# ipc-sim/IPC

Measured on NVIDIA H100. Metric: newton_iteration_ms_assembly_ccd, lower is better.
Workload: dtype f64

## Files before the change

### ipc_b200/csrc/api_mesh.cu

```cuda
#include "abi.h"
#include <algorithm>
#include <cmath>
#include <numeric>
#include <vector>

using namespace ipcgpu;

int build_maps(ipcgpu_ctx* ctx)
{
    const int nT = ctx->nT, nV = ctx->nV;
    const std::vector<int>& T = ctx->h_T;
    ctx->t_begin = (int)((int64_t)nT * ctx->rank / ctx->nranks);
    ctx->t_end = (int)((int64_t)nT * (ctx->rank + 1) / ctx->nranks);
    std::vector<int64_t> cum(nV + 1, 0);
    for (size_t i = 0; i < (size_t)4 * nT; ++i) ++cum[T[i] + 1];
    for (int v = 0; v < nV; ++v) cum[v + 1] += cum[v];
    auto boundary = [&](int r) -> int {
        if (r <= 0) return 0;
        if (r >= ctx->nranks) return nV;
        const int64_t target = cum[nV] * r / ctx->nranks;
        return (int)(std::lower_bound(cum.begin(), cum.end(), target) - cum.begin());
    };
    const int vb = std::min(boundary(ctx->rank), nV), ve = std::max(vb, std::min(boundary(ctx->rank + 1), nV));
    ctx->v_begin = vb;
    ctx->v_end = ve;
    std::vector<int> list;
    if (ctx->nranks == 1) {
        list.resize(nT);
        std::iota(list.begin(), list.end(), 0);
    }
    else {
        list.reserve((size_t)(nT / ctx->nranks) + 1024);
        for (int t = 0; t < nT; ++t) {
            bool touch = false;
            for (int k = 0; k < 4; ++k) {
                const int v = T[(size_t)k * nT + t];
                touch = touch || (v >= vb && v < ve);
            }
            if (touch) list.push_back(t);
        }
    }
    const int nL = (int)list.size();
    ctx->n_list = nL;
    if (list.empty()) list.push_back(0);
    REQUIRE(ctx->tet_list.upload(list.data(), list.size(), ctx->stream), IPCGPU_ERR_CUDA, "upload of the tet list failed");
    std::vector<int> ptr(nV + 1, 0);
    for (int l = 0; l < nL; ++l)
        for (int k = 0; k < 4; ++k) {
            const int v = T[(size_t)k * nT + list[l]];
            if (v >= vb && v < ve) ++ptr[v + 1];
        }
    for (int v = 0; v < nV; ++v) ptr[v + 1] += ptr[v];
    std::vector<int> inc((size_t)std::max(ptr[nV], 1)), cur(ptr.begin(), ptr.end() - 1);
    for (int l = 0; l < nL; ++l)
        for (int k = 0; k < 4; ++k) {
            const int v = T[(size_t)k * nT + list[l]];
            if (v >= vb && v < ve) inc[cur[v]++] = 4 * l + k;
        }
    if (!ctx->inc_ptr.upload(ptr.data(), ptr.size(), ctx->stream) || !ctx->inc.upload(inc.data(), inc.size(), ctx->stream)) {
        ctx->err = "upload of incidence map failed";
        return IPCGPU_ERR_CUDA;
    }
    REQUIRE(((uint64_t)nL + 64ull) * 78ull < 0xffffffffull, IPCGPU_ERR_CAPACITY, "local tet count too large for 32-bit block offsets");
    struct KS {
        uint64_t key;
        unsigned src;
        unsigned tet;
    };
    std::vector<KS> ks;
    ks.reserve((size_t)10 * nL);
    static const int pa[6] = { 0, 0, 0, 1, 1, 2 }, pb[6] = { 1, 2, 3, 2, 3, 3 };
    for (int l = 0; l < nL; ++l) {
        const int t = list[l];
        int v[4];
        for (int k = 0; k < 4; ++k) v[k] = T[(size_t)k * nT + t];
        const unsigned tl = (unsigned)l, tile_base = (tl / 64u) * (64u * 78u), tin = tl % 64u;
        for (int a = 0; a < 4; ++a)
            if (v[a] >= vb && v[a] < ve) ks.push_back({ ((uint64_t)v[a] << 32) | (uint32_t)v[a], tile_base + 6u * a * 64u + tin * 6u, tl });
        for (int q = 0; q < 6; ++q) {
            const int lo = std::min(v[pa[q]], v[pb[q]]), hi = std::max(v[pa[q]], v[pb[q]]);
            if (lo >= vb && lo < ve) ks.push_back({ ((uint64_t)lo << 32) | (uint32_t)hi, tile_base + (24u + 9u * q) * 64u + tin * 9u, tl });
        }
    }
    std::sort(ks.begin(), ks.end(), [](const KS& a, const KS& b) { return a.key < b.key || (a.key == b.key && (a.tet < b.tet || (a.tet == b.tet && a.src < b.src))); });
    std::vector<int> sv, su, cptr;
    std::vector<unsigned> csrc(std::max<size_t>(ks.size(), 1));
    for (size_t i = 0; i < ks.size(); ++i) {
        if (i == 0 || ks[i].key != ks[i - 1].key) {
            sv.push_back((int)(ks[i].key >> 32));
            su.push_back((int)(ks[i].key & 0xffffffffu));
            cptr.push_back((int)i);
        }
        csrc[i] = ks[i].src;
    }
    cptr.push_back((int)ks.size());
    {
        const size_t nS = sv.size();
        std::vector<int> order;
        order.reserve(nS);
        for (size_t i = 0; i < nS; ++i)
            if (sv[i] != su[i]) order.push_back((int)i);
        ctx->nOffSlots = (int)order.size();
        for (size_t i = 0; i < nS; ++i)
            if (sv[i] == su[i]) order.push_back((int)i);
        std::vector<int> sv2(nS), su2(nS), cptr2;
        std::vector<unsigned> csrc2(csrc.size());
        cptr2.reserve(nS + 1);
        size_t pos = 0;
        for (size_t k = 0; k < nS; ++k) {
            const int i = order[k];
            sv2[k] = sv[i];
            su2[k] = su[i];
            cptr2.push_back((int)pos);
            for (int c = cptr[i]; c < cptr[i + 1]; ++c) csrc2[pos++] = csrc[c];
        }
        cptr2.push_back((int)pos);
        sv.swap(sv2); su.swap(su2); cptr.swap(cptr2); csrc.swap(csrc2);
    }
    ctx->nSlots = (int)sv.size();
    if (sv.empty()) { sv.push_back(0); su.push_back(0); }
    bool ok = ctx->slot_v.upload(sv.data(), sv.size(), ctx->stream) && ctx->slot_u.upload(su.data(), su.size(), ctx->stream)
        && ctx->con_ptr.upload(cptr.data(), cptr.size(), ctx->stream) && ctx->con_src.upload(csrc.data(), csrc.size(), ctx->stream)
        && ctx->slot_off.reserve((size_t)3 * std::max(1, ctx->nSlots));
    REQUIRE(ok, IPCGPU_ERR_CUDA, "upload of Hessian scatter map failed");
    ALLOC(ctx->gcont, (size_t)12 * std::max(1, nL));
    ALLOC(ctx->hblk, (size_t)78 * 64 * ((size_t)(std::max(1, nL) + 63) / 64));
    ALLOC(ctx->partials, (size_t)std::max(1, elastic_energy_blocks(ctx->t_end - ctx->t_begin)) + 8);
    CK(cudaStreamSynchronize(ctx->stream));
    ctx->maps_ready = true;
    ctx->offsets_ready = false;
    ctx->damp_on = ctx->damp_inc_ready = ctx->nbc_on = false;
    ctx->n_dbc = 0;
    for (int slot : { kEnergyDamping, kEnergyNeumann, kEnergyDirichlet })
        CK(cudaMemsetAsync(&ctx->iter.p->energy[slot], 0, sizeof(double), ctx->stream));
    CK(cudaStreamSynchronize(ctx->stream));
    return IPCGPU_OK;
}

void owned_value_range(ipcgpu_ctx* ctx)
{
    if (ctx->h_ia.empty()) return;
    ctx->a_begin = (long long)ctx->h_ia[(size_t)3 * ctx->v_begin] - ctx->index_base;
    ctx->a_end = (long long)ctx->h_ia[(size_t)3 * ctx->v_end] - ctx->index_base;
}

int ensure_offsets(ipcgpu_ctx* ctx)
{
    if (ctx->offsets_ready) return IPCGPU_OK;
    REQUIRE(ctx->maps_ready, IPCGPU_ERR_STATE, "ipcgpu_set_mesh must precede Hessian assembly");
    REQUIRE(ctx->n_rows == 3 * ctx->nV, IPCGPU_ERR_STATE, "ipcgpu_set_csr must be called with n_rows = 3*nV");
    CK(cudaMemsetAsync(ctx->flag.p, 0, sizeof(int), ctx->stream));
    slot_offsets(ctx->nSlots, ctx->slot_v.p, ctx->slot_u.p, ctx->ia.p, ctx->ja.p, ctx->index_base, ctx->slot_off.p, ctx->flag.p, ctx->stream);
    ++ctx->launches;
    int h = 0;
    CK(cudaMemcpyAsync(&h, ctx->flag.p, sizeof(int), cudaMemcpyDeviceToHost, ctx->stream));
    CK(cudaStreamSynchronize(ctx->stream));
    REQUIRE(h == 0, IPCGPU_ERR_PATTERN, "CSR pattern misses a block of the mesh topology (row<=col entries of every tet vertex pair are required)");
    ctx->offsets_ready = true;
    return IPCGPU_OK;
}

int upload_dir(ipcgpu_ctx* ctx, const double* p)
{
    if (p) {
        CK(cudaMemcpyAsync(ctx->dir.p, p, (size_t)3 * ctx->nV * sizeof(double), cudaMemcpyHostToDevice, ctx->stream));
        double pSize = 0;
        int nMeshSV = 0;
        for (int i = 0; i < ctx->nSV; ++i) {
            const int v = ctx->h_SVI[i];
            if (v >= ctx->nVdof) continue;
            ++nMeshSV;
            pSize += std::abs(p[3 * (size_t)v]);
            pSize += std::abs(p[3 * (size_t)v + 1]);
            pSize += std::abs(p[3 * (size_t)v + 2]);
        }
        ctx->pSize = nMeshSV > 0 ? pSize / (double)((long long)nMeshSV * 3) : 0.0;
        ALLOC(ctx->pSize_dev, 1);
        ctx->staging->pSize = ctx->pSize;
        CK(cudaMemcpyAsync(ctx->pSize_dev.p, &ctx->staging->pSize, sizeof(double), cudaMemcpyHostToDevice, ctx->stream));
        ctx->pSize_surface = ctx->surface_ready;
        ctx->dir_valid = true;
    }
    REQUIRE(ctx->dir_valid, IPCGPU_ERR_STATE, "no search direction uploaded yet");
    return IPCGPU_OK;
}
// ... 76 lines not shown
int ipcgpu_save_state(ipcgpu_ctx* ctx)
{
    REQUIRE(ctx->nV > 0, IPCGPU_ERR_STATE, "ipcgpu_set_mesh first");
    ENTER(kSerial);
    CK(cudaMemcpyAsync(ctx->Vsaved.p, ctx->V.p, (size_t)3 * ctx->nV * sizeof(double), cudaMemcpyDeviceToDevice, ctx->stream));
    ctx->state_saved = true;
    return IPCGPU_OK;
}

int ipcgpu_set_search_dir(ipcgpu_ctx* ctx, const double* p)
{
    REQUIRE(ctx->nV > 0 && p, IPCGPU_ERR_ARG, "ipcgpu_set_search_dir: mesh and p required");
    ENTER(kSerial);
    return upload_dir(ctx, p);
}

int ipcgpu_step_forward(ipcgpu_ctx* ctx, const double* p, double alpha)
{
    REQUIRE(ctx->nV > 0, IPCGPU_ERR_STATE, "ipcgpu_set_mesh first");
    REQUIRE(ctx->state_saved, IPCGPU_ERR_STATE, "ipcgpu_save_state must precede ipcgpu_step_forward");
    ENTER(kSerial);
    int rc = upload_dir(ctx, p);
    if (rc) return rc;
    step_forward(ctx->nV, ctx->Vsaved.p, ctx->dir.p, alpha, ctx->V.p, ctx->stream);
    ++ctx->launches;
    CK(cudaGetLastError());
    ctx->mark_inputs();
    return IPCGPU_OK;
}

int ipcgpu_elastic_energy(ipcgpu_ctx* ctx, double coef, int , double* E)
{
    REQUIRE(ctx->maps_ready, IPCGPU_ERR_STATE, "ipcgpu_set_mesh first");
    ENTER(kSerial);
    cudaEvent_t pe = ctx->prof_begin(IPCGPU_STAGE_ELASTIC_ENERGY);
    elastic_energy(ctx->eargs(), ctx->e_per_tet.p, ctx->partials.p, ctx->stream);
    return energy_tail(ctx, kEnergyElastic, ctx->partials.p, elastic_energy_blocks(ctx->t_end - ctx->t_begin), coef, pe, E);
}

static int zero_values(ipcgpu_ctx* ctx)
{
    cudaStream_t st = ctx->deriv_stream();
    if (ctx->device_pattern) {
        const bool owned = ctx->nranks > 1 && !ctx->a_all_dirty;
        zero_csr_rows(ctx->ia.p, ctx->index_base, owned ? 3 * ctx->v_begin : 0, owned ? 3 * ctx->v_end : 3 * ctx->nV, ctx->a.p, st);
    }
    else if (ctx->nranks > 1 && !ctx->a_all_dirty) {
        if (ctx->a_end > ctx->a_begin) zero_words(ctx->a.p + ctx->a_begin, (size_t)(ctx->a_end - ctx->a_begin) * 2, st);
    }
    else zero_words(ctx->a.p, (size_t)ctx->nnz * 2, st);
    ++ctx->launches;
    CK(cudaGetLastError());
    ctx->a_all_dirty = false;
    return IPCGPU_OK;
}

static int run_grad_hess(ipcgpu_ctx* ctx, double coef, int projectSPD, int projectDBC, bool need_g, bool need_h, int add_mass, bool with_energy = false,
    bool cleared = false)
{
    REQUIRE(ctx->maps_ready, IPCGPU_ERR_STATE, "ipcgpu_set_mesh first");
    if (need_h) {
        int rc = ensure_offsets(ctx);
        if (rc) return rc;
    }
    cudaStream_t st = ctx->deriv_stream();
    cudaEvent_t pe = ctx->prof_begin(IPCGPU_STAGE_ELASTIC_TET);
    double* e_part = nullptr;
    if (with_energy) {
        ALLOC(ctx->e_partials2, (size_t)elastic_grad_hess_blocks(ctx->n_list) + 8);
        e_part = ctx->e_partials2.p;
    }
    elastic_grad_hess(ctx->eargs(), coef, projectSPD, need_g, need_h, ctx->gcont.p, ctx->hblk.p, st, e_part);
    ctx->hblk_valid = need_h;
    ctx->prof_end(pe);
    ++ctx->launches;
    if (with_energy) {
        pe = ctx->prof_begin(IPCGPU_STAGE_ELASTIC_ENERGY);
        reduce_sum(e_part, elastic_grad_hess_blocks(ctx->n_list), coef, &ctx->iter.p->energy[kEnergyElastic], st);
        ctx->prof_end(pe);
        ++ctx->launches;
    }
    if (need_g) {
        pe = ctx->prof_begin(IPCGPU_STAGE_GATHER_GRADIENT);
        gather_gradient(ctx->nV, ctx->inc_ptr.p, ctx->inc.p, ctx->gcont.p, ctx->has_dbc ? ctx->dbc.p : nullptr, projectDBC, 0, ctx->g.p, st);
        ctx->prof_end(pe);
        ++ctx->launches;
    }
    if (need_h) {
        pe = ctx->prof_begin(IPCGPU_STAGE_ASSEMBLE_CSR);
        assemble_csr(ctx->nOffSlots, ctx->nSlots, ctx->slot_v.p, ctx->slot_u.p, ctx->slot_off.p, ctx->con_ptr.p, ctx->con_src.p, ctx->hblk.p,
            ctx->has_dbc ? ctx->dbc.p : nullptr, projectDBC, nullptr, cleared ? 0 : 1, ctx->a.p, st);
        const double* m = (add_mass && ctx->has_mass) ? ctx->mass.p : nullptr;
        diag_mass_dbc_range(ctx->v_begin, ctx->v_end, ctx->ia.p, ctx->index_base, ctx->has_dbc ? ctx->dbc.p : nullptr, projectDBC, m, ctx->a.p, st);
        ctx->prof_end(pe);
        ctx->launches += 2;
    }
    CK(cudaGetLastError());
    return IPCGPU_OK;
}

int ipcgpu_elastic_gradient(ipcgpu_ctx* ctx, double coef, int , int projectDBC, double* g)
{
    ENTER(g ? kSerial : kDerivative);
    int rc = run_grad_hess(ctx, coef, 1, projectDBC, true, false, 0);
    return rc || !g ? rc : gradient_roundtrip_end(ctx, g);
}

int ipcgpu_elastic_hessian(ipcgpu_ctx* ctx, double coef, int , int projectSPD, int projectDBC, double* a_inout)
{
    int rc = hessian_begin(ctx, kDerivative, a_inout);
    if (rc || (rc = run_grad_hess(ctx, coef, projectSPD, projectDBC, false, true, 0))) return rc;
    return hessian_end(ctx, a_inout, 0);
}

static int elastic_derivatives(ipcgpu_ctx* ctx, double coef, int projectSPD, int projectDBC, int add_mass, bool with_energy, double* E, double* g, double* a)
{
    REQUIRE(ctx->nnz > 0, IPCGPU_ERR_STATE, "ipcgpu_set_csr first");
    ENTER(E || g || a ? kSerial : kDerivative);
    int rc = a ? sync_pattern_mirror(ctx) : 0;
    if (rc || (rc = zero_values(ctx))) return rc;
    if ((rc = run_grad_hess(ctx, coef, projectSPD, projectDBC, true, true, add_mass, with_energy, true))) return rc;
    if (ctx->nranks > 1 && (g || a)) {
        rc = ipcgpu_allreduce_grad_hess(ctx, g ? 1 : 0, a ? 1 : 0);
        if (rc) return rc;
    }
    if (g) CK(cudaMemcpyAsync(g, ctx->g.p, (size_t)3 * ctx->nV * sizeof(double), cudaMemcpyDeviceToHost, ctx->stream));
    if (a) CK(cudaMemcpyAsync(a, ctx->a.p, (size_t)ctx->nnz * sizeof(double), cudaMemcpyDeviceToHost, ctx->stream));
    if (with_energy && (rc = energy_result(ctx, kEnergyElastic, E))) return rc;
    if (!E && (g || a)) CK(cudaStreamSynchronize(ctx->stream));
    return IPCGPU_OK;
}

int ipcgpu_elastic_grad_hess(ipcgpu_ctx* ctx, double coef, int projectSPD, int projectDBC, int add_mass, double* g, double* a)
{
    return elastic_derivatives(ctx, coef, projectSPD, projectDBC, add_mass, false, nullptr, g, a);
}

int ipcgpu_elastic_energy_grad_hess(ipcgpu_ctx* ctx, double coef, int projectSPD, int projectDBC, int add_mass, double* E, double* g, double* a)
{
    return elastic_derivatives(ctx, coef, projectSPD, projectDBC, add_mass, true, E, g, a);
}

int ipcgpu_step_bound_set(ipcgpu_ctx* ctx, double alpha)
{
    REQUIRE(alpha >= 0.0, IPCGPU_ERR_ARG, "the step must be non-negative");
    ENTER(kStepBound);
    step_set(ctx->iter.p, alpha, ctx->stream);
    ++ctx->launches;
    CK(cudaGetLastError());
    return IPCGPU_OK;
}

int ipcgpu_inversion_step(ipcgpu_ctx* ctx, const double* p, double slack, double* alpha_inout)
{
    REQUIRE(ctx->maps_ready, IPCGPU_ERR_STATE, "ipcgpu_set_mesh first");
    ENTER(p || alpha_inout ? kSerial : kStepBound);
    int rc = upload_dir(ctx, p);
    if (rc) return rc;
    if (alpha_inout && (rc = ipcgpu_step_bound_set(ctx, *alpha_inout))) return rc;
    cudaEvent_t pe = ctx->prof_begin(IPCGPU_STAGE_INVERSION);
    inversion_step(ctx->eargs(), ctx->dir.p, slack, ctx->inv_steps.p, ctx->iter.p, ctx->stream);
    ctx->prof_end(pe);
    ctx->launches += 2;
    if ((rc = nccl_min_u64(ctx, &ctx->iter.p->inv_ord))) return rc;
    inversion_apply(ctx->iter.p, ctx->nT, ctx->stream);
    ++ctx->launches;
    CK(cudaGetLastError());
    if (alpha_inout) return ccd_read_back(ctx, alpha_inout);
    return IPCGPU_OK;
}

static int solve_pcg(ipcgpu_ctx* ctx, bool multilevel, const double* rhs, double rel_tol, int max_iter, double* x, int adopt_as_search_dir, int* iters, double* rel_residual)
{
    REQUIRE(ctx->nnz > 0 && ctx->n_rows == 3 * ctx->nV, IPCGPU_ERR_STATE, "ipcgpu_set_csr first");
// ... 70 lines not shown
```

### ipc_b200/csrc/context.h

```cpp
#pragma once
#include "kernels.h"
#include "broadphase_types.h"
#include <cuda_runtime.h>
#include <cstdint>
#include <cstring>
#include <string>
#include <vector>

namespace ipcgpu {

template <typename T>
struct DevBuf {
    T* p = nullptr;
    size_t n = 0;
    ~DevBuf() { release(); }
    void release()
    {
        if (p) cudaFree(p);
        p = nullptr;
        n = 0;
    }
    bool reserve(size_t count)
    {
        if (count <= n) return true;
// ... 115 lines not shown
    int hs_count[2];
};

}

struct ipcgpu_ctx {
    int device = 0;
    cudaStream_t stream = nullptr;
    cudaStream_t deriv = nullptr;
    cudaEvent_t ev_deriv_fork = nullptr, ev_deriv_done = nullptr;
    bool deriv_open = false, deriv_copied = false;
    int prio_low = 0, prio_high = 0;
    cudaStream_t deriv_stream() const { return deriv_open ? deriv : stream; }
    cudaStream_t side = nullptr;
    cudaStream_t copy = nullptr;
    cudaEvent_t ev_copy_fork = nullptr, ev_copy_join = nullptr;
    bool copy_pending = false;
    cudaEvent_t ev_inputs = nullptr, ev_join = nullptr, ev_scatter = nullptr;
    bool scatter_marked = false;
    bool inputs_marked = false;
    void mark_inputs()
    {
        inputs_marked = (cudaEventRecord(ev_inputs, stream) == cudaSuccess);
    }
    std::string err;
    uint64_t launches = 0;

    int rank = 0, nranks = 1;
    void* nccl_comm = nullptr;
    int v_begin = 0, v_end = 0, n_list = 0;
    ipcgpu::DevBuf<int> tet_list;
    long long a_begin = 0, a_end = 0;

    ipcgpu::DevBuf<ipcgpu::IterState> iter;
    ipcgpu::IterState* h_iter = nullptr;
    double pSize = 0.0;
    bool dir_valid = false, pSize_surface = false;
    unsigned local_scalars = 0;
    bool a_all_dirty = false;
    std::vector<int> h_ia;

    int nV = 0, nT = 0, energy = 0;
    int t_begin = 0, t_end = 0;
    ipcgpu::DevBuf<double> V, Vsaved, Vrest, Ainv, vol, mu, lam, mass, Vprev, xtilde;
    bool prev_set = false, xtilde_set = false;
    ipcgpu::DevBuf<int> T;
    ipcgpu::DevBuf<uint8_t> dbc;
    bool has_mass = false, has_dbc = false, state_saved = false;
    std::vector<int> h_T;

    int nSV = 0, nSE = 0, nSF = 0;
    int nVdof = 0x7fffffff;
    int ee_as_vf = 1;
    ipcgpu::DevBuf<int> SVI, SE, SF, vCoDim;
    bool has_codim = false, surface_ready = false;
    int pair_capacity = 1 << 20;
    int exchange_capacity = 1 << 16;
    bool canonical_order = true;
    bool partition_contact = false, lists_local = false;
    ipcgpu::ContactWork cw;
    ipcgpu::CcdWork ccd;
    ipcgpu::PointTetWork pit;
    int n_hs = 0;
    ipcgpu::DevBuf<double> hs_par, hs_lam, hs_partials;
    ipcgpu::DevBuf<int> hs_flags, hs_offs, hs_cnt, hs_pstart;
    ipcgpu::DevBuf<int2> hs_act, hs_lag;
    ipcgpu::DevBuf<unsigned char> hs_scan;
    size_t hs_scan_bytes = 0;
    bool hs_set_built = false, hs_lag_ready = false;
    bool damp_on = false, damp_inc_ready = false, nbc_on = false;
    int n_dbc = 0;
    ipcgpu::DevBuf<double> damp_D, damp_partials, nbc_f, nbc_partials, dbc_tgt, dbc_lam, dbc_partials;
    ipcgpu::DevBuf<int> damp_inc_ptr, damp_inc, dbc_vid;
    ipcgpu::DevBuf<ipcgpu::TimeParams> tparams;
    ipcgpu::DevBuf<double> vel, acc, dxe;
    bool time_set = false;
    int dyn_nV = 0;
    size_t ccd_capacity = (size_t)1 << 23;
    std::vector<int> h_SVI;
    double debug_prune_seed = -1.0;
    long long debug_ti_budget = -1;

    ipcgpu::DevBuf<int> inc_ptr, inc;
    int nSlots = 0, nOffSlots = 0;
    ipcgpu::DevBuf<int> slot_v, slot_u, slot_off, con_ptr;
    ipcgpu::DevBuf<unsigned> con_src;
    bool hblk_valid = false;
    bool maps_ready = false, offsets_ready = false;

    int n_rows = 0, nnz = 0, index_base = 0;
    ipcgpu::DevBuf<int> ia, ja;
    ipcgpu::DevBuf<double> a;
    ipcgpu::DevBuf<int> flag;
    bool device_pattern = false, pat_pending = false;
    uint64_t pat_seen_version = 0;
    int pat_changed_host = 0;
    ipcgpu::PatternWork pw;
    ipcgpu::DevBuf<int> fia, fja, fpos;
    bool full_pattern_ready = false;
    ipcgpu::DevBuf<double> sol, pcg_b, pcg_r, pcg_p, pcg_q, pcg_minv, pcg_scal, pcg_hist;
    ipcgpu::MultilevelWork ml;

    ipcgpu::DevBuf<double> gcont, hblk, g, e_per_tet, partials, inv_steps, dir, in_partials, e_partials2;
    ipcgpu::DevBuf<double> packed_scalars;
    ipcgpu::DevBuf<double> pSize_dev;

    struct HostState {
        unsigned local_scalars;
        bool lists_local, lists_global, want_cand, swept_ready, fr_ready, inputs_marked, scatter_marked, hs_set_built, hs_lag_ready;
        int nC, nP, nK, fr_host_n;
    };
    struct GraphRec {
        cudaGraphExec_t exec = nullptr;
        cudaGraph_t graph = nullptr;
        uint64_t launches = 0, epoch = 0;
        bool dirty_at_begin = false;
        bool updates_pattern = false;
        bool step_control = false;
        std::vector<cudaGraph_t> bodies;
        HostState hs;
    };
    std::vector<GraphRec> graphs;
    std::vector<cudaGraph_t> capture_bodies;
    static constexpr int kCondDepth = 3;
    cudaStream_t cond_streams[kCondDepth] = { nullptr, nullptr, nullptr };
    int cond_depth = 0;
    bool sc_pending = false, sc_pending_at_capture = false;
    bool capturing = false, pat_pending_at_capture = false;
    uint64_t epoch = 0, launches_at_capture = 0;
    bool dirty_at_capture = false;
    ipcgpu::HostStaging* staging = nullptr;

    bool profiling = false;
    std::vector<std::pair<cudaEvent_t, cudaEvent_t>> prof[16];
    cudaEvent_t timer_a = nullptr, timer_b = nullptr;
    cudaEvent_t prof_begin(int stage)
    {
        if (!profiling) return nullptr;
        cudaEvent_t a, b;
        cudaEventCreate(&a);
        cudaEventCreate(&b);
        prof[stage].emplace_back(a, b);
        cudaEventRecord(a, stream);
        return b;
    }
    void prof_end(cudaEvent_t b)
    {
        if (b) cudaEventRecord(b, stream);
    }

    ipcgpu::ElasticArgs eargs() const
    {
        ipcgpu::ElasticArgs p;
        p.nV = nV; p.nT = nT; p.t_begin = t_begin; p.t_end = t_end;
        p.n_list = n_list; p.tet_list = (nranks > 1) ? tet_list.p : nullptr;
        p.V = V.p; p.T = T.p; p.Ainv = Ainv.p; p.vol = vol.p; p.mu = mu.p; p.lam = lam.p; p.energy = energy;
        p.e_row_lo = (nranks > 1) ? v_begin : 0; p.e_row_hi = (nranks > 1) ? v_end : nV;
        return p;
    }
};
```

### ipc_b200/csrc/elastic.cu

```cuda
#include "elastic.cuh"
#include "kernels.h"

namespace ipcgpu {

constexpr int kHessTile = 64;

struct TetIn {
    int v[4];
    double x[4][3];
    M3 A;
    double vol, mu, lam;
};

DEV void load_tet(const ElasticArgs& p, int t, TetIn& in)
{
#pragma unroll
    for (int k = 0; k < 4; ++k) in.v[k] = __ldg(p.T + (size_t)k * p.nT + t);
#pragma unroll
    for (int k = 0; k < 4; ++k)
#pragma unroll
        for (int c = 0; c < 3; ++c) in.x[k][c] = __ldg(p.V + (size_t)c * p.nV + in.v[k]);
#pragma unroll
    for (int q = 0; q < 9; ++q) in.A.m[q] = __ldg(p.Ainv + (size_t)q * p.nT + t);
    in.vol = __ldg(p.vol + t);
// ... 180 lines not shown
                    Ht(2, 1) = a12 * wa2 * wb1 + o12 * wa1 * wb2;
                    M3 Tm;
#pragma unroll
                    for (int i = 0; i < 3; ++i)
#pragma unroll
                        for (int m = 0; m < 3; ++m) Tm(i, m) = U(i, 0) * Ht(0, m) + U(i, 1) * Ht(1, m) + U(i, 2) * Ht(2, m);
                    double* oo = buf + tx * len;
                    if (a == b) {
                        int q = 0;
#pragma unroll
                        for (int i = 0; i < 3; ++i)
#pragma unroll
                            for (int r = i; r < 3; ++r) oo[q++] = Tm(i, 0) * U(r, 0) + Tm(i, 1) * U(r, 1) + Tm(i, 2) * U(r, 2);
                    }
                    else {
                        const bool flip = in.v[a] > in.v[b];
#pragma unroll
                        for (int i = 0; i < 3; ++i)
#pragma unroll
                            for (int r = 0; r < 3; ++r) {
                                double h = Tm(i, 0) * U(r, 0) + Tm(i, 1) * U(r, 1) + Tm(i, 2) * U(r, 2);
                                oo[flip ? (3 * r + i) : (3 * i + r)] = h;
                            }
                    }
                }
                asm volatile("fence.proxy.async.shared::cta;\n" ::: "memory");
                __syncthreads();
                if (tx == 0 && ntile > 0) {
                    tma_store_tile(hblk + (size_t)tileI * (kHessTile * 78) + (size_t)o * kHessTile, buf, (unsigned)ntile * (unsigned)len * 8u);
                    asm volatile("cp.async.bulk.wait_group.read 1;\n" ::: "memory");
                }
                __syncthreads();
                ++slot;
            }
        }
    }
    asm volatile("fence.proxy.async.shared::cta;\n" ::: "memory");
    __syncthreads();
    if (tx == 0) {
        if (NEED_G && ntile > 0) tma_store_tile(gcont + (size_t)tile0 * 12, sG, (unsigned)ntile * 12u * 8u);
        asm volatile("cp.async.bulk.wait_group.read 0;\n" ::: "memory");
    }
    if (e_partials) {
        __shared__ double sE[2];
        const double ws = warp_sum(e_tet);
        if ((threadIdx.x & 31) == 0) sE[threadIdx.x >> 5] = ws;
        __syncthreads();
        if (threadIdx.x == 0) {
            double acc = 0.0;
#pragma unroll
            for (int i = 0; i < 2; ++i) acc += sE[i];
            e_partials[blockIdx.x] = acc;
        }
    }
}

__global__ void __launch_bounds__(256) k_gather_gradient(int nV, const int* __restrict__ inc_ptr, const int* __restrict__ inc ,
    const double* __restrict__ gcont, const uint8_t* __restrict__ dbc, int projectDBC, int accumulate, double* __restrict__ g)
{
    const int v = blockIdx.x * blockDim.x + threadIdx.x;
    if (v >= nV) return;
    double gx = 0.0, gy = 0.0, gz = 0.0;
    const int e = inc_ptr[v + 1];
    for (int q = inc_ptr[v]; q < e; ++q) {
        const int id = __ldg(inc + q);
        const double* s = gcont + (size_t)(id >> 2) * 12 + 3 * (id & 3);
        gx += s[0];
        gy += s[1];
        gz += s[2];
    }
    if (projectDBC && dbc && dbc[v]) gx = gy = gz = 0.0;
    if (accumulate) {
        g[3 * (size_t)v] += gx;
        g[3 * (size_t)v + 1] += gy;
        g[3 * (size_t)v + 2] += gz;
    }
    else {
        g[3 * (size_t)v] = gx;
        g[3 * (size_t)v + 1] = gy;
        g[3 * (size_t)v + 2] = gz;
    }
}

__global__ void __launch_bounds__(288) k_assemble_csr(int nOff, int nSlots, const int* __restrict__ slot_v, const int* __restrict__ slot_u,
    const int* __restrict__ slot_off , const int* __restrict__ con_ptr, const unsigned* __restrict__ con_src,
    const double* __restrict__ hblk, const uint8_t* __restrict__ dbc, int projectDBC, const double* __restrict__ mass,
    int accumulate, double* __restrict__ a)
{
    const long long tid = (long long)blockIdx.x * blockDim.x + threadIdx.x, tOff = 9ll * nOff;
    int sIdx, q;
    if (tid < tOff) {
        sIdx = (int)(tid / 9);
        q = (int)(tid - 9ll * sIdx);
    }
    else {
        const int k = (int)((tid - tOff) / 6);
        sIdx = nOff + k;
        q = (int)(tid - tOff - 6ll * k);
    }
    if (sIdx >= nSlots) return;
    const int v = slot_v[sIdx], u = slot_u[sIdx];
    const bool diag = (v == u);
    if (diag && q >= 6) return;
    const bool pv = dbc && (dbc[v] == 1 || (dbc[v] == 2 && projectDBC));
    const bool pu = dbc && (dbc[u] == 1 || (dbc[u] == 2 && projectDBC));
    const bool dropped = pv || pu;
    double h = 0.0;
    if (!dropped) {
        const int b = con_ptr[sIdx], e = con_ptr[sIdx + 1];
#pragma unroll 4
        for (int k = b; k < e; ++k) h += hblk[__ldg(con_src + k) + q];
    }
    int r, c;
    if (diag) { r = (q < 3) ? 0 : (q < 5 ? 1 : 2); c = (q < 3) ? q : (q < 5 ? q - 3 : 0); }
    else { r = q / 3; c = q - 3 * r; }
    const int o = slot_off[3 * sIdx + r] + c;
    if (accumulate) {
        if (!dropped) a[o] += h;
        else if (diag) a[o] = 0.0;
    }
    else a[o] = h;
    (void)mass;
}

__global__ void __launch_bounds__(256) k_diag_mass_dbc(int v0, int nV, const int* __restrict__ ia, int base, const uint8_t* __restrict__ dbc, int projectDBC,
    const double* __restrict__ mass, double* __restrict__ a)
{
    const int v = v0 + blockIdx.x * blockDim.x + threadIdx.x;
    if (v >= nV) return;
    const bool pv = dbc && (dbc[v] == 1 || (dbc[v] == 2 && projectDBC));
#pragma unroll
    for (int r = 0; r < 3; ++r) {
        const int o = ia[3 * v + r] - base;
        if (pv) a[o] = 1.0;
        else if (mass) a[o] += mass[v];
    }
}

__global__ void __launch_bounds__(256) k_slot_offsets(int nSlots, const int* __restrict__ slot_v, const int* __restrict__ slot_u,
    const int* __restrict__ ia, const int* __restrict__ ja, int base, int* __restrict__ slot_off, int* __restrict__ err, const int* __restrict__ gate)
{
    const int sIdx = blockIdx.x * blockDim.x + threadIdx.x;
    if (sIdx >= nSlots || (gate && !*gate)) return;
    const int v = slot_v[sIdx], u = slot_u[sIdx];
#pragma unroll
    for (int r = 0; r < 3; ++r) {
        const int row = 3 * v + r;
        const int col = (v == u) ? row : 3 * u;
        int lo = ia[row] - base, hi = ia[row + 1] - base;
        const int target = col + base;
        int found = -1;
        while (lo < hi) {
            int mid = (lo + hi) >> 1;
            int c = ja[mid];
            if (c < target) lo = mid + 1;
            else hi = mid;
        }
        if (lo < ia[row + 1] - base && ja[lo] == target) found = lo;
        if (found < 0) atomicExch(err, 1);
        slot_off[3 * sIdx + r] = found;
    }
}

struct Cplx {
    double re, im;
};
DEV Cplx cmul(Cplx a, Cplx b) { return { a.re * b.re - a.im * b.im, a.re * b.im + a.im * b.re }; }
DEV Cplx cdiv(Cplx a, Cplx b)
{
    if (fabs(b.re) >= fabs(b.im)) {
        double r = b.im / b.re, den = b.re + b.im * r;
        return { (a.re + a.im * r) / den, (a.im - a.re * r) / den };
    }
    else {
        double r = b.re / b.im, den = b.re * r + b.im;
        return { (a.re * r + a.im) / den, (a.im * r - a.re) / den };
    }
}
DEV Cplx csqrt_(Cplx z)
{
    if (z.re == 0.0 && z.im == 0.0) return { 0.0, z.im };
    double m = hypot(z.re, z.im);
    if (z.re >= 0.0) {
        double t = sqrt(0.5 * (m + z.re));
        return { t, z.im / (2.0 * t) };
    }
    else {
        double t = sqrt(0.5 * (m - z.re));
        return { fabs(z.im) / (2.0 * t), copysign(t, z.im) };
    }
}
DEV Cplx cpow_third(Cplx z)
{
    if (z.im == 0.0 && z.re > 0.0) return { pow(z.re, 1.0 / 3.0), 0.0 };
    if (z.re == 0.0 && z.im == 0.0) return { 0.0, 0.0 };
    double lr = log(hypot(z.re, z.im)), th = atan2(z.im, z.re);
    double rho = exp((1.0 / 3.0) * lr), ang = (1.0 / 3.0) * th;
    return { rho * cos(ang), rho * sin(ang) };
}
DEV double quad_root(double a, double b, double c, double tol)
{
    double t;
    if (fabs(a) <= tol) t = -c / b;
    else {
        double desc = b * b - 4 * a * c;
// ... 59 lines not shown
        const int tt = p.t_begin + t;
        int v[4];
#pragma unroll
        for (int k = 0; k < 4; ++k) v[k] = __ldg(p.T + (size_t)k * p.nT + tt);
        double x[4][3], d[4][3];
#pragma unroll
        for (int k = 0; k < 4; ++k)
#pragma unroll
            for (int c = 0; c < 3; ++c) {
                x[k][c] = __ldg(p.V + (size_t)c * p.nV + v[k]);
                d[k][c] = __ldg(dir + 3 * (size_t)v[k] + c);
            }
        double e[3][3], f[3][3];
#pragma unroll
        for (int k = 0; k < 3; ++k)
#pragma unroll
            for (int c = 0; c < 3; ++c) {
                e[k][c] = x[k + 1][c] - x[0][c];
                f[k][c] = d[k + 1][c] - d[0][c];
            }
        const double ca = det3v(f[0], f[1], f[2]);
        const double cb = det3v(e[0], f[1], f[2]) + det3v(f[0], e[1], f[2]) + det3v(f[0], f[1], e[2]);
        const double cc = det3v(f[0], e[1], e[2]) + det3v(e[0], f[1], e[2]) + det3v(e[0], e[1], f[2]);
        const double cd = (1.0 - slack) * det3v(e[0], e[1], e[2]);
        const double r = cubic_root(ca, cb, cc, cd, 1.0e-6);
        out = (r >= 0) ? r : 1e20;
        if (per_tet) per_tet[tt] = out;
    }
    double m = warp_min(__dadd_rn(out, 0.0));
    __shared__ double sm[8];
    if ((threadIdx.x & 31) == 0) sm[threadIdx.x >> 5] = m;
    __syncthreads();
    if (threadIdx.x == 0) {
        double mm = sm[0];
#pragma unroll
        for (int i = 1; i < 8; ++i) mm = fmin(mm, sm[i]);
        atomicMin(min_ord, dbl_to_ord(mm));
    }
}

void elastic_energy(const ElasticArgs& p, double* e_per_tet, double* partials, cudaStream_t st)
{
    const int nb = elastic_energy_blocks(p.t_end - p.t_begin);
    if (nb <= 0) return;
    if (p.energy == 0) k_elastic_energy<0><<<nb, 256, 0, st>>>(p, e_per_tet, partials);
    else k_elastic_energy<1><<<nb, 256, 0, st>>>(p, e_per_tet, partials);
}
int elastic_energy_blocks(int nTets) { return (nTets + 255) / 256; }
void reduce_sum(const double* partials, int n, double scale, double* out, cudaStream_t st) { k_reduce_sum<<<1, 1024, 0, st>>>(partials, n, scale, out); }

int elastic_grad_hess_blocks(int n_list) { return (n_list + kHessTile - 1) / kHessTile; }
template <int ENERGY, bool G, bool H>
static void launch_gh(const ElasticArgs& p, double coef, int projectSPD, double* gcont, double* hblk, cudaStream_t st, double* e_partials)
{
    const int n = p.n_list;
    if (n <= 0) return;
    const size_t smem = (size_t)kHessTile * 8 * ((H ? 18 : 0) + (G ? 12 : 0));
    static bool attr_set = false;
    if (!attr_set) {
        cudaFuncSetAttribute(k_elastic_grad_hess<ENERGY, G, H>, cudaFuncAttributeMaxDynamicSharedMemorySize, (int)smem);
        attr_set = true;
    }
    k_elastic_grad_hess<ENERGY, G, H><<<elastic_grad_hess_blocks(n), kHessTile, smem, st>>>(p, coef, projectSPD, gcont, hblk, e_partials);
}
void elastic_grad_hess(const ElasticArgs& p, double coef, int projectSPD, bool need_g, bool need_h, double* gcont, double* hblk, cudaStream_t st, double* e_partials)
{
    if (p.energy == 0) {
        if (need_g && need_h) launch_gh<0, true, true>(p, coef, projectSPD, gcont, hblk, st, e_partials);
        else if (need_g) launch_gh<0, true, false>(p, coef, projectSPD, gcont, hblk, st, e_partials);
        else if (need_h) launch_gh<0, false, true>(p, coef, projectSPD, gcont, hblk, st, e_partials);
    }
    else {
        if (need_g && need_h) launch_gh<1, true, true>(p, coef, projectSPD, gcont, hblk, st, e_partials);
        else if (need_g) launch_gh<1, true, false>(p, coef, projectSPD, gcont, hblk, st, e_partials);
        else if (need_h) launch_gh<1, false, true>(p, coef, projectSPD, gcont, hblk, st, e_partials);
    }
}

void gather_gradient(int nV, const int* inc_ptr, const int* inc, const double* gcont, const uint8_t* dbc, int projectDBC, int accumulate, double* g, cudaStream_t st)
{
    if (nV <= 0) return;
    k_gather_gradient<<<(nV + 255) / 256, 256, 0, st>>>(nV, inc_ptr, inc, gcont, dbc, projectDBC, accumulate, g);
}
void assemble_csr(int nOff, int nSlots, const int* slot_v, const int* slot_u, const int* slot_off, const int* con_ptr, const unsigned* con_src,
    const double* hblk, const uint8_t* dbc, int projectDBC, const double* mass, int accumulate, double* a, cudaStream_t st)
{
    if (nSlots <= 0) return;
    const int nb = (int)(((long long)nOff * 9 + (long long)(nSlots - nOff) * 6 + 287) / 288);
    k_assemble_csr<<<nb, 288, 0, st>>>(nOff, nSlots, slot_v, slot_u, slot_off, con_ptr, con_src, hblk, dbc, projectDBC, mass, accumulate, a);
}
void diag_mass_dbc(int nV, const int* ia, int base, const uint8_t* dbc, int projectDBC, const double* mass, double* a, cudaStream_t st)
{
    if (nV > 0 && (dbc || mass)) k_diag_mass_dbc<<<(nV + 255) / 256, 256, 0, st>>>(0, nV, ia, base, dbc, projectDBC, mass, a);
}
void diag_mass_dbc_range(int v0, int v1, const int* ia, int base, const uint8_t* dbc, int projectDBC, const double* mass, double* a, cudaStream_t st)
{
    if (v1 > v0 && (dbc || mass)) k_diag_mass_dbc<<<(v1 - v0 + 255) / 256, 256, 0, st>>>(v0, v1, ia, base, dbc, projectDBC, mass, a);
}
void slot_offsets(int nSlots, const int* slot_v, const int* slot_u, const int* ia, const int* ja, int base, int* slot_off, int* err, cudaStream_t st, const int* gate)
{
    if (nSlots <= 0) return;
    k_slot_offsets<<<(nSlots + 255) / 256, 256, 0, st>>>(nSlots, slot_v, slot_u, ia, ja, base, slot_off, err, gate);
}
void inversion_step(const ElasticArgs& p, const double* dir, double slack, double* per_tet, IterState* st_dev, cudaStream_t st)
{
    k_inversion_init<<<1, 32, 0, st>>>(st_dev);
    const int n = p.t_end - p.t_begin;
    if (n <= 0) return;
    k_inversion_step<<<(n + 255) / 256, 256, 0, st>>>(p, dir, slack, per_tet, &st_dev->inv_ord);
}
void inversion_apply(IterState* st_dev, int nT, cudaStream_t st) { k_inversion_apply<<<1, 32, 0, st>>>(st_dev, nT); }
void step_set(IterState* st_dev, double alpha, cudaStream_t st) { k_step_set<<<1, 32, 0, st>>>(st_dev, alpha); }

constexpr int kFlags = kEnergySlots, kChecks = kFlags + 8, kCrossings = kChecks + 2;
static_assert(kCrossings + 1 == kPackedScalars && kPackedScalars <= 32, "one warp packs the scalars");
__global__ void k_pack_scalars(const IterState* __restrict__ st, unsigned local_mask, double* __restrict__ buf)
{
    const int i = threadIdx.x;
    if (i < kFlags) buf[i] = ((local_mask >> i) & 1u) ? st->energy[i] : 0.0;
    else if (i < kChecks) buf[i] = (double)st->flags[i - kFlags];
    else if (i < kCrossings) buf[i] = (local_mask & kLocalChecks) ? (double)st->checks[i - kChecks] : 0.0;
    else if (i == kCrossings) buf[i] = (local_mask & kLocalCrossings) ? (double)st->hs_crossings : 0.0;
}
__global__ void k_unpack_scalars(IterState* __restrict__ st, unsigned local_mask, const double* __restrict__ buf)
{
    const int i = threadIdx.x;
    if (i < kFlags) { if ((local_mask >> i) & 1u) st->energy[i] = buf[i]; }
    else if (i < kChecks) st->flags[i - kFlags] = (int)fmin(buf[i], 2147483647.0);
    else if (i < kCrossings) { if (local_mask & kLocalChecks) st->checks[i - kChecks] = (int)buf[i]; }
    else if (i == kCrossings) { if (local_mask & kLocalCrossings) st->hs_crossings = (int)buf[i]; }
}
void pack_scalars(const IterState* st_dev, unsigned local_mask, double* buf, cudaStream_t st) { k_pack_scalars<<<1, 32, 0, st>>>(st_dev, local_mask, buf); }
void unpack_scalars(IterState* st_dev, unsigned local_mask, const double* buf, cudaStream_t st) { k_unpack_scalars<<<1, 32, 0, st>>>(st_dev, local_mask, buf); }

}
```

### ipc_b200/csrc/kernels.h

```cpp
#pragma once
#include <cuda_runtime.h>
#include <cstdint>

namespace ipcgpu {

enum { kEnergyElastic = 0, kEnergyBarrier, kEnergyFriction, kEnergyInertia, kEnergyPlaneBarrier, kEnergyPlaneFriction, kEnergyDamping, kEnergyNeumann,
    kEnergyDirichlet, kEnergySlots };

struct IterState {
    unsigned long long step_ord;
    unsigned long long inv_ord;
    unsigned long long ccd_ord;
    unsigned long long cand_range[2];
    unsigned long long n_full_cand;
    double max_t;
    double alpha_grid;
    double ref_lo[3], ref_inv_h;
    double alpha_stage[4];
    double energy[kEnergySlots];
    int ref_count[3];
    int n_set[3];
    int flags[8];
    int grid_axis_cells;
    int pad_;
    int checks[2];
    unsigned long long ccd_stats[8];
    unsigned long long sc_pmax_ord;
    double sc_alpha_cfl;
    double ls_E0, ls_Et, ls_LF;
    int sc_full_ccd;
    int sc_status;
    int ls_count[4];
    int ls_stopped, ls_rebuilt, ls_post_ran;
    int ls_cond;
    double dbc_rho;
    double dbc_step;
    double dbc_tol;
    double nbc_coef;
    double hs_alpha;
    int hs_n_active, hs_n_lagged;
    int hs_crossings;
    int hs_zero_step;
    long long pat_nnz;
    unsigned long long pat_version;
    int pat_changed;
    int pat_ok;
    int pat_diff;
    int pat_pad_;
};
enum { kCflBranch = 0, kCflClamp, kLsEntry, kLsStart, kLsInversion, kLsIntersection, kLsArmijo, kLsPostCheck, kLsPostLoop, kLsRebuild, kWsEntry };
enum { kTermInertia = 1, kTermFriction = 2, kTermHalfSpace = 4, kTermHalfSpaceFriction = 8, kTermDamping = 16, kTermNeumann = 32, kTermDirichlet = 64 };
enum { FLAG_NONPOSITIVE_DISTANCE = 0, FLAG_SET_CAPACITY = 1, FLAG_CCD_CAPACITY = 2, FLAG_ZERO_CCD_DISTANCE = 3, FLAG_PATTERN = 4, FLAG_TI_WARNINGS = 5, FLAG_EXCHANGE_CAPACITY = 6,
    FLAG_PATTERN_CAPACITY = 7 };
enum : unsigned { kLocalChecks = 1u << kEnergySlots, kLocalCrossings = 1u << (kEnergySlots + 1) };
constexpr int kPackedScalars = kEnergySlots + 8 + 2 + 1;

struct ElasticArgs {
    int nV, nT;
    int t_begin, t_end;
    int n_list;
    const int* tet_list;
    const double* V;
    const int* T;
    const double* Ainv;
    const double* vol;
    const double* mu;
    const double* lam;
    int energy;
    int e_row_lo, e_row_hi;
};

void elastic_energy(const ElasticArgs& p, double* e_per_tet, double* partials, cudaStream_t st);
int elastic_energy_blocks(int nTets);
void elastic_grad_hess(const ElasticArgs& p, double coef, int projectSPD, bool need_g, bool need_h, double* gcont, double* hblk, cudaStream_t st, double* e_partials = nullptr);
int elastic_grad_hess_blocks(int n_list);
void gather_gradient(int nV, const int* inc_ptr, const int* inc, const double* gcont, const uint8_t* dbc, int projectDBC, int accumulate, double* g, cudaStream_t st);
void assemble_csr(int nOff, int nSlots, const int* slot_v, const int* slot_u, const int* slot_off, const int* con_ptr, const unsigned* con_src,
    const double* hblk, const uint8_t* dbc, int projectDBC, const double* mass, int accumulate, double* a, cudaStream_t st);
void diag_mass_dbc(int nV, const int* ia, int base, const uint8_t* dbc, int projectDBC, const double* mass, double* a, cudaStream_t st);
void slot_offsets(int nSlots, const int* slot_v, const int* slot_u, const int* ia, const int* ja, int base, int* slot_off, int* err, cudaStream_t st,
    const int* gate = nullptr);
void diag_mass_dbc_range(int v0, int v1, const int* ia, int base, const uint8_t* dbc, int projectDBC, const double* mass, double* a, cudaStream_t st);
void inversion_step(const ElasticArgs& p, const double* dir, double slack, double* per_tet, IterState* st_dev, cudaStream_t st);
void inversion_apply(IterState* st_dev, int nT, cudaStream_t st);
void step_set(IterState* st_dev, double alpha, cudaStream_t st);
void pack_scalars(const IterState* st_dev, unsigned local_mask, double* buf, cudaStream_t st);
void unpack_scalars(IterState* st_dev, unsigned local_mask, const double* buf, cudaStream_t st);


struct SurfArgs {
    int nV;
    const double* V;
    const double* Vrest;
    const uint8_t* dbc;
    const int* vCoDim;
    int nSV; const int* SVI;
    int nSE; const int* SE;
    int nSF; const int* SF;
    int nVdof, ee_as_vf;
};
__device__ __forceinline__ bool obstacle_vertex(const SurfArgs& s, int v) { return v >= s.nVdof; }

struct BarrierArgs {
    int nV;
    const double* V;
    const double* Vrest;
    const uint8_t* dbc;
    const int* SE;
    const int4* cs; const int* nC;
    const int4* para; const int2* para_e; const int* nP;
    int rank, nranks, share;
    int row_lo, row_hi;
    double dHat, kappa;
    int projectDBC;
    const int* ia; const int* ja; int base;
    int nVdof;
};

void barrier_energy(const BarrierArgs& p, double* partials, int* bad, cudaStream_t st);
int barrier_energy_blocks();
void barrier_gradient(const BarrierArgs& p, double* g, cudaStream_t st);
void evaluate_constraints(const BarrierArgs& p, double* val, cudaStream_t st);
void constraint_jacobian_t(const BarrierArgs& p, const double* input, double coef, double* g, cudaStream_t st);
void para_gradient(const BarrierArgs& p, double* g, cudaStream_t st);
void barrier_hessian_build_project(const BarrierArgs& p, int* flags, double* Hraw, int* rows, int* psd, int* n_owned, int capacity, cudaStream_t st);
void barrier_hessian_scatter(const BarrierArgs& p, double* a, int* flags, const double* Hraw, const int* rows, const int* psd, const int* n_owned, int capacity, cudaStream_t st);
struct FrictionArgs {
    int nV;
    const double* V;
    const double* Vt;
    const uint8_t* dbc;
    const int4* cs; const int* n;
    const double* lambda;
    const double2* coord;
    const double* basis;
    double eps2, coef;
    int projectDBC;
    const int* ia; const int* ja; int base;
    int rank, nranks;
    int row_lo, row_hi;
};
void friction_lag(const BarrierArgs& p, int4* cs_out, int* n_out, double* lambda, double2* coord, double* basis, int capacity, int* bad, cudaStream_t st);
void friction_energy(const FrictionArgs& p, double* partials, cudaStream_t st);
int friction_energy_blocks();
void friction_gradient(const FrictionArgs& p, double* g, cudaStream_t st);
void friction_hessian(const FrictionArgs& p, double* a, int* err, cudaStream_t st);
void zero_csr_rows(const int* ia, int base, int row0, int row1, double* a, cudaStream_t st);
void reduce_sum(const double* partials, int n, double scale, double* out, cudaStream_t st);

void step_forward(int nV, const double* x0_soa, const double* p_interleaved, double alpha, double* x_soa, cudaStream_t st,
    const unsigned long long* alpha_ord = nullptr);
void cfl_pmax(int nSV, const int* SVI, int nVdof, const double* dir, IterState* st_dev, cudaStream_t st);
void step_decide(IterState* st_dev, int op, double a, int b, unsigned long long handle, cudaStream_t st);
int inertia_energy_blocks(int nV);
void inertia_energy(int v0, int v1, int nV, const double* x_soa, const double* xtilde_soa, const double* mass, double* partials, cudaStream_t st);
void inertia_gradient(int nV, const double* x_soa, const double* xtilde_soa, const double* mass, const uint8_t* dbc, int projectDBC, double* g, cudaStream_t st);
constexpr int kPlaneStride = 8;
constexpr int kMaxPlanes = 8;
struct HalfSpaceArgs {
    int nV, nSV, nP;
    const int* SVI;
// ... 79 lines not shown
```

Measured before the change: 2.798.

## Fuse gradient gather into CSR assembly with shared-memory staged contribution lists

The separate gradient gather kernel is replaced, when the Hessian is also needed, by extra threads in the CSR assembly kernel. Diagonal slots use their otherwise idle lanes 6-8 to sum gradient contributions, remapping each Hessian source index to its gcont location. The assembly kernel now works on 32-slot blocks, stages the contribution index list in shared memory and prefetches values in batches of four. This removes one kernel launch and its separate incidence traversal. The cost is a zero-fill of g, shared-memory traffic, and a hard-coded index mapping that ties the gradient layout to the Hessian block layout.

```diff
diff --git a/ipc_b200/csrc/api_mesh.cu b/ipc_b200/csrc/api_mesh.cu
--- a/ipc_b200/csrc/api_mesh.cu
+++ b/ipc_b200/csrc/api_mesh.cu
@@ -100,7 +100,6 @@
         order.reserve(nS);
         for (size_t i = 0; i < nS; ++i)
             if (sv[i] != su[i]) order.push_back((int)i);
-        ctx->nOffSlots = (int)order.size();
         for (size_t i = 0; i < nS; ++i)
             if (sv[i] == su[i]) order.push_back((int)i);
         std::vector<int> sv2(nS), su2(nS), cptr2;
@@ -343,14 +342,15 @@
     }
     if (need_g) {
         pe = ctx->prof_begin(IPCGPU_STAGE_GATHER_GRADIENT);
-        gather_gradient(ctx->nV, ctx->inc_ptr.p, ctx->inc.p, ctx->gcont.p, ctx->has_dbc ? ctx->dbc.p : nullptr, projectDBC, 0, ctx->g.p, st);
+        if (need_h) zero_words(ctx->g.p, (size_t)6 * ctx->nV, st);
+        else gather_gradient(ctx->nV, ctx->inc_ptr.p, ctx->inc.p, ctx->gcont.p, ctx->has_dbc ? ctx->dbc.p : nullptr, projectDBC, 0, ctx->g.p, st);
         ctx->prof_end(pe);
         ++ctx->launches;
     }
     if (need_h) {
         pe = ctx->prof_begin(IPCGPU_STAGE_ASSEMBLE_CSR);
-        assemble_csr(ctx->nOffSlots, ctx->nSlots, ctx->slot_v.p, ctx->slot_u.p, ctx->slot_off.p, ctx->con_ptr.p, ctx->con_src.p, ctx->hblk.p,
-            ctx->has_dbc ? ctx->dbc.p : nullptr, projectDBC, nullptr, cleared ? 0 : 1, ctx->a.p, st);
+        assemble_csr(ctx->nSlots, ctx->slot_v.p, ctx->slot_u.p, ctx->slot_off.p, ctx->con_ptr.p, ctx->con_src.p, ctx->hblk.p, ctx->gcont.p,
+            ctx->has_dbc ? ctx->dbc.p : nullptr, projectDBC, cleared ? 0 : 1, ctx->a.p, need_g ? ctx->g.p : nullptr, st);
         const double* m = (add_mass && ctx->has_mass) ? ctx->mass.p : nullptr;
         diag_mass_dbc_range(ctx->v_begin, ctx->v_end, ctx->ia.p, ctx->index_base, ctx->has_dbc ? ctx->dbc.p : nullptr, projectDBC, m, ctx->a.p, st);
         ctx->prof_end(pe);
diff --git a/ipc_b200/csrc/context.h b/ipc_b200/csrc/context.h
--- a/ipc_b200/csrc/context.h
+++ b/ipc_b200/csrc/context.h
@@ -221,7 +221,7 @@
     long long debug_ti_budget = -1;
 
     ipcgpu::DevBuf<int> inc_ptr, inc;
-    int nSlots = 0, nOffSlots = 0;
+    int nSlots = 0;
     ipcgpu::DevBuf<int> slot_v, slot_u, slot_off, con_ptr;
     ipcgpu::DevBuf<unsigned> con_src;
     bool hblk_valid = false;
diff --git a/ipc_b200/csrc/elastic.cu b/ipc_b200/csrc/elastic.cu
--- a/ipc_b200/csrc/elastic.cu
+++ b/ipc_b200/csrc/elastic.cu
@@ -286,45 +286,93 @@
     }
 }
 
-__global__ void __launch_bounds__(288) k_assemble_csr(int nOff, int nSlots, const int* __restrict__ slot_v, const int* __restrict__ slot_u,
+constexpr int kAsmSlots = 32;
+constexpr int kAsmThreads = 9 * kAsmSlots;
+constexpr int kAsmStage = 2048;
+constexpr int kAsmBatch = 4;
+constexpr unsigned kAsmDiag = 1, kAsmDropped = 2, kAsmGradZero = 4;
+
+DEV unsigned diag_block_to_gcont(unsigned o)
+{
+    const unsigned tile = o / (64u * 78u), r = o - tile * (64u * 78u), a = r / 384u, tin = (r - 384u * a) / 6u;
+    return tile * (64u * 12u) + 12u * tin + 3u * a;
+}
+
+template <bool GRAD>
+DEV void load_batch(const unsigned* src, int k, int e, const double* __restrict__ base, double (&x)[kAsmBatch])
+{
+#pragma unroll
+    for (int j = 0; j < kAsmBatch; ++j) {
+        const unsigned o = src[min(k + j, e - 1)];
+        x[j] = __ldg(base + (GRAD ? diag_block_to_gcont(o) : o));
+    }
+}
+
+template <bool GRAD>
+DEV double sum_contributions(const unsigned* src, int k, int e, const double* __restrict__ base)
+{
+    double h = 0.0;
+    if (k >= e) return h;
+    double x[kAsmBatch];
+    load_batch<GRAD>(src, k, e, base, x);
+    for (; k < e; k += kAsmBatch) {
+        double y[kAsmBatch];
+        if (k + kAsmBatch < e) load_batch<GRAD>(src, k + kAsmBatch, e, base, y);
+#pragma unroll
+        for (int j = 0; j < kAsmBatch; ++j)
+            if (k + j < e) h += x[j];
+#pragma unroll
+        for (int j = 0; j < kAsmBatch; ++j) x[j] = y[j];
+    }
+    return h;
+}
+
+__global__ void __launch_bounds__(kAsmThreads) k_assemble_csr(int nSlots, const int* __restrict__ slot_v, const int* __restrict__ slot_u,
     const int* __restrict__ slot_off , const int* __restrict__ con_ptr, const unsigned* __restrict__ con_src,
-    const double* __restrict__ hblk, const uint8_t* __restrict__ dbc, int projectDBC, const double* __restrict__ mass,
-    int accumulate, double* __restrict__ a)
-{
-    const long long tid = (long long)blockIdx.x * blockDim.x + threadIdx.x, tOff = 9ll * nOff;
-    int sIdx, q;
-    if (tid < tOff) {
-        sIdx = (int)(tid / 9);
-        q = (int)(tid - 9ll * sIdx);
-    }
-    else {
-        const int k = (int)((tid - tOff) / 6);
-        sIdx = nOff + k;
-        q = (int)(tid - tOff - 6ll * k);
-    }
-    if (sIdx >= nSlots) return;
-    const int v = slot_v[sIdx], u = slot_u[sIdx];
-    const bool diag = (v == u);
-    if (diag && q >= 6) return;
-    const bool pv = dbc && (dbc[v] == 1 || (dbc[v] == 2 && projectDBC));
-    const bool pu = dbc && (dbc[u] == 1 || (dbc[u] == 2 && projectDBC));
-    const bool dropped = pv || pu;
+    const double* __restrict__ hblk, const double* __restrict__ gcont, const uint8_t* __restrict__ dbc, int projectDBC, int accumulate,
+    double* __restrict__ a, double* __restrict__ g)
+{
+    __shared__ unsigned sSrc[kAsmStage];
+    __shared__ int sPtr[kAsmSlots + 1], sV[kAsmSlots], sOff[3 * kAsmSlots];
+    __shared__ unsigned sFlags[kAsmSlots];
+    const int tx = threadIdx.x, s0 = (gridDim.x - 1 - blockIdx.x) * kAsmSlots, nS = min(kAsmSlots, nSlots - s0);
+    const int cb = __ldg(con_ptr + s0), n = __ldg(con_ptr + s0 + nS) - cb;
+    const bool staged = n <= kAsmStage;
+    if (staged)
+        for (int i = tx; i < n; i += kAsmThreads) sSrc[i] = __ldg(con_src + cb + i);
+    if (tx <= nS) sPtr[tx] = __ldg(con_ptr + s0 + tx) - cb;
+    if (tx < 3 * nS) sOff[tx] = __ldg(slot_off + 3 * s0 + tx);
+    if (tx < nS) {
+        const int v = __ldg(slot_v + s0 + tx), u = __ldg(slot_u + s0 + tx);
+        const bool pv = dbc && (dbc[v] == 1 || (dbc[v] == 2 && projectDBC));
+        const bool pu = dbc && (dbc[u] == 1 || (dbc[u] == 2 && projectDBC));
+        sV[tx] = v;
+        sFlags[tx] = (v == u ? kAsmDiag : 0u) | (pv || pu ? kAsmDropped : 0u) | (projectDBC && dbc && dbc[v] ? kAsmGradZero : 0u);
+    }
+    __syncthreads();
+    const int j = tx / 9, q = tx - 9 * j;
+    if (j >= nS) return;
+    const unsigned f = sFlags[j];
+    const bool diag = f & kAsmDiag, grad = diag && q >= 6;
+    if (grad && !g) return;
+    const int b = sPtr[j], e = sPtr[j + 1];
     double h = 0.0;
-    if (!dropped) {
-        const int b = con_ptr[sIdx], e = con_ptr[sIdx + 1];
-#pragma unroll 4
-        for (int k = b; k < e; ++k) h += hblk[__ldg(con_src + k) + q];
-    }
+    if (grad) h = staged ? sum_contributions<true>(sSrc, b, e, gcont + (q - 6)) : sum_contributions<true>(con_src + cb, b, e, gcont + (q - 6));
+    else if (!(f & kAsmDropped)) h = staged ? sum_contributions<false>(sSrc, b, e, hblk + q) : sum_contributions<false>(con_src + cb, b, e, hblk + q);
+    if (grad) {
+        g[3 * (size_t)sV[j] + (q - 6)] = (f & kAsmGradZero) ? 0.0 : h;
+        return;
+    }
+    const bool dropped = f & kAsmDropped;
     int r, c;
     if (diag) { r = (q < 3) ? 0 : (q < 5 ? 1 : 2); c = (q < 3) ? q : (q < 5 ? q - 3 : 0); }
     else { r = q / 3; c = q - 3 * r; }
-    const int o = slot_off[3 * sIdx + r] + c;
+    const int o = sOff[3 * j + r] + c;
     if (accumulate) {
         if (!dropped) a[o] += h;
         else if (diag) a[o] = 0.0;
     }
     else a[o] = h;
-    (void)mass;
 }
 
 __global__ void __launch_bounds__(256) k_diag_mass_dbc(int v0, int nV, const int* __restrict__ ia, int base, const uint8_t* __restrict__ dbc, int projectDBC,
@@ -550,12 +598,12 @@
     if (nV <= 0) return;
     k_gather_gradient<<<(nV + 255) / 256, 256, 0, st>>>(nV, inc_ptr, inc, gcont, dbc, projectDBC, accumulate, g);
 }
-void assemble_csr(int nOff, int nSlots, const int* slot_v, const int* slot_u, const int* slot_off, const int* con_ptr, const unsigned* con_src,
-    const double* hblk, const uint8_t* dbc, int projectDBC, const double* mass, int accumulate, double* a, cudaStream_t st)
+void assemble_csr(int nSlots, const int* slot_v, const int* slot_u, const int* slot_off, const int* con_ptr, const unsigned* con_src,
+    const double* hblk, const double* gcont, const uint8_t* dbc, int projectDBC, int accumulate, double* a, double* g, cudaStream_t st)
 {
     if (nSlots <= 0) return;
-    const int nb = (int)(((long long)nOff * 9 + (long long)(nSlots - nOff) * 6 + 287) / 288);
-    k_assemble_csr<<<nb, 288, 0, st>>>(nOff, nSlots, slot_v, slot_u, slot_off, con_ptr, con_src, hblk, dbc, projectDBC, mass, accumulate, a);
+    k_assemble_csr<<<(nSlots + kAsmSlots - 1) / kAsmSlots, kAsmThreads, 0, st>>>(nSlots, slot_v, slot_u, slot_off, con_ptr, con_src, hblk, gcont, dbc,
+        projectDBC, accumulate, a, g);
 }
 void diag_mass_dbc(int nV, const int* ia, int base, const uint8_t* dbc, int projectDBC, const double* mass, double* a, cudaStream_t st)
 {
diff --git a/ipc_b200/csrc/kernels.h b/ipc_b200/csrc/kernels.h
--- a/ipc_b200/csrc/kernels.h
+++ b/ipc_b200/csrc/kernels.h
@@ -75,8 +75,8 @@
 void elastic_grad_hess(const ElasticArgs& p, double coef, int projectSPD, bool need_g, bool need_h, double* gcont, double* hblk, cudaStream_t st, double* e_partials = nullptr);
 int elastic_grad_hess_blocks(int n_list);
 void gather_gradient(int nV, const int* inc_ptr, const int* inc, const double* gcont, const uint8_t* dbc, int projectDBC, int accumulate, double* g, cudaStream_t st);
-void assemble_csr(int nOff, int nSlots, const int* slot_v, const int* slot_u, const int* slot_off, const int* con_ptr, const unsigned* con_src,
-    const double* hblk, const uint8_t* dbc, int projectDBC, const double* mass, int accumulate, double* a, cudaStream_t st);
+void assemble_csr(int nSlots, const int* slot_v, const int* slot_u, const int* slot_off, const int* con_ptr, const unsigned* con_src,
+    const double* hblk, const double* gcont, const uint8_t* dbc, int projectDBC, int accumulate, double* a, double* g, cudaStream_t st);
 void diag_mass_dbc(int nV, const int* ia, int base, const uint8_t* dbc, int projectDBC, const double* mass, double* a, cudaStream_t st);
 void slot_offsets(int nSlots, const int* slot_v, const int* slot_u, const int* ia, const int* ja, int base, int* slot_off, int* err, cudaStream_t st,
     const int* gate = nullptr);
diff --git a/profiles/assembly_timing.py b/profiles/assembly_timing.py
--- /dev/null
+++ b/profiles/assembly_timing.py
@@ -0,0 +1,64 @@
+import argparse
+import hashlib
+import json
+import os
+import sys
+
+import numpy as np
+
+ROOT = os.path.dirname(os.path.dirname(os.path.abspath(__file__)))
+sys.path.insert(0, ROOT)
+sys.path.insert(0, os.path.join(ROOT, "profiles"))
+
+import bench
+from device_pattern_timing import Args, gpu_info, med
+from ipc_b200 import lib as L
+
+
+def main():
+    ap = argparse.ArgumentParser()
+    ap.add_argument("--reps", type=int, default=10)
+    ap.add_argument("--calls", type=int, default=20)
+    args = ap.parse_args()
+    m, info = bench.build_scene(Args())
+    ctx = L.Context(0)
+    ctx.set_mesh(m.V_rest_soa, m.T_soa, m.restTriInv, m.vol, m.mu, m.lam, m.mass, m.dbc, m.energy)
+    ctx.set_surface(m.SVI, m.SFEdges, m.SF_soa, m.vCoDim)
+    ctx.set_state(m.V_soa)
+    mm, pa, pe, _ = ctx.constraint_set(info["dHat"], 1)
+    ia, ja = m.csr_pattern(1, extra_pairs=bench.contact_pattern_pairs(m, mm, pa, pe))
+    ctx.set_csr(ia, ja, 1)
+    out = {"gpu": gpu_info(), "scene": f"C5, {m.nT} tets, {m.nV} vertices, nnz {ja.size}", "calls": args.calls, "reps": args.reps}
+
+    def chain():
+        for _ in range(args.calls):
+            ctx.elastic_energy_grad_hess(bench.DT2, 1, 1, 1, None, None)
+
+    chain()
+    ctx.sync()
+    t = []
+    for _ in range(args.reps):
+        ctx.timer_start()
+        chain()
+        t.append(ctx.timer_stop() / args.calls)
+    out["chain_ms_per_call"] = {"median": med(t), "min_max": [min(t), max(t)]}
+
+    ctx.profile(1)
+    chain()
+    ctx.sync()
+    prof = ctx.profile_read()
+    ctx.profile(0)
+    stages = {k: prof[k][0] / args.calls for k in ("elastic_tet", "gather_gradient", "assemble_csr") if k in prof}
+    stages["gather_gradient+assemble_csr"] = stages.get("gather_gradient", 0.0) + stages.get("assemble_csr", 0.0)
+    out["eager_stage_ms_per_call"] = stages
+
+    g, a = np.empty(3 * m.nV), np.empty(ja.size)
+    ctx.elastic_energy_grad_hess(bench.DT2, 1, 1, 1, g, a)
+    out["sha256"] = {"gradient": hashlib.sha256(g.tobytes()).hexdigest(), "csr_values": hashlib.sha256(a.tobytes()).hexdigest()}
+    out["gpu_after"] = gpu_info()
+    print(json.dumps(out))
+    ctx.close()
+
+
+if __name__ == "__main__":
+    main()
```

Result: faster. 2.744 (median of 6 runs) (-1.9%).
